# razayunus/ManhattanSLAM

Hardware: AMD Instinct MI355X
Metric: RGB-D frames/sec at 640x480 (ORB+surfel front end) (higher is better)
Workload: dtype u8/i32 (ORB)/f32+f64 (surfel)

## Files before the change

### manhattanslam_amd/csrc/msl_sf_superpixel.hip

```cpp

#include "msl_sf.h"

using namespace msl;
using namespace msl::sf;

namespace {

__device__ __forceinline__ double div100_exact(double x) {
    const double y = 0.01;
    const double q0 = x * y;
    const double q1 = fma(fma(-q0, 100.0, x), y, q0);
    return fma(fma(-q1, 100.0, x), y, q1);
}

constexpr float float_below(float f) { return __builtin_bit_cast(float, __builtin_bit_cast(unsigned, f) - 1u); }
constexpr float HUBER_RANGE_F = (float)HUBER_RANGE, MAX_ANGLE_COS_F = (float)MAX_ANGLE_COS, DEPTH_005_F = 0.05f, DEPTH_01_F = 0.1f;
static_assert((double)HUBER_RANGE_F > HUBER_RANGE && (double)float_below(HUBER_RANGE_F) < HUBER_RANGE, "0.4f is the float next above 0.4");
static_assert((double)MAX_ANGLE_COS_F > MAX_ANGLE_COS && (double)float_below(MAX_ANGLE_COS_F) < MAX_ANGLE_COS, "0.1f is the float next above 0.1");
static_assert((double)DEPTH_005_F > 0.05 && (double)float_below(DEPTH_005_F) < 0.05, "0.05f is the float next above 0.05");
static_assert((double)DEPTH_01_F > 0.1 && (double)float_below(DEPTH_01_F) < 0.1, "0.1f is the float next above 0.1");
__device__ __forceinline__ bool in_huber_band(float r) { return r < HUBER_RANGE_F && r > -HUBER_RANGE_F; }

__device__ __forceinline__ float seq_sum_f32(const float *a, int n, float s) {
    int p = 0;
    for (; p + 8 <= n; p += 8) {
        const float4 u = *reinterpret_cast<const float4 *>(a + p), v = *reinterpret_cast<const float4 *>(a + p + 4);
        s += u.x; s += u.y; s += u.z; s += u.w; s += v.x; s += v.y; s += v.z; s += v.w;
    }
    for (; p < n; p++) s += a[p];
    return s;
}
__device__ __forceinline__ float huber_term_add(float s, float t) {
    return __builtin_isinf(t) ? (float)((double)s + (t > 0 ? HUBER_RANGE : -1 * HUBER_RANGE)) : s + t;
}

__device__ __forceinline__ float row_ror1(float v) {
    return __int_as_float(__builtin_amdgcn_update_dpp(0, __float_as_int(v), 0x121, 0xF, 0xF, false));
}
__device__ __forceinline__ float chain_block_f32(float s, float t) {
#pragma unroll
    for (int q = 0; q < 16; q++) s = row_ror1(s) + t;
    return s;
}
__device__ __forceinline__ float chain_block_huber(float s, float t) {
#pragma unroll
    for (int q = 0; q < 16; q++) s = huber_term_add(row_ror1(s), t);
    return s;
}

__global__ __launch_bounds__(256) void kb_seed_init(SfDev P) {
    const int slot = blockIdx.y;
    const int seedI = blockIdx.x * 256 + threadIdx.x;
    if (seedI >= P.nseeds) return;
    if (seedI == 0) P.wlCount[slot] = 0;
    const FrameDev F = P.frames[slot];
    const int spX = seedI % P.spW, spY = seedI / P.spW;
    int imageX = spX * SP + SP / 2, imageY = spY * SP + SP / 2;
    imageX = imageX < (P.W - 1) ? imageX : (P.W - 1);
    imageY = imageY < (P.H - 1) ? imageY : (P.H - 1);
    msl_seed s;
    memset(&s, 0, sizeof(s));
    P.fused[(size_t)slot * P.flagStride + seedI] = 0;
    if (member_at(P, F, imageY, imageX) != -1) {
        P.seeds[(size_t)slot * P.nseeds + seedI] = s; P.arec[(size_t)slot * P.nseeds + seedI] = assign_rec(s);
        return;
    }
    s.use = 1;
    s.x = (float)imageX; s.y = (float)imageY;
    vec3b(P, F, (float)imageY, (float)imageX, s.r, s.g, s.b);
    s.meanIntensity = gray_at(P, F, imageY, imageX);
    s.meanDepth = depth_at(P, F, imageY, imageX);
    if (s.meanDepth < 0.01) {
        int xb = spX * SP + SP / 2 - SP, yb = spY * SP + SP / 2 - SP;
        int xe = xb + SP * 2, ye = yb + SP * 2;
        xb = xb > 0 ? xb : 0; yb = yb > 0 ? yb : 0;
        xe = xe < P.W - 1 ? xe : P.W - 1; ye = ye < P.H - 1 ? ye : P.H - 1;
        bool found = false;
        for (int j = yb; j < ye && !found; j++)
            for (int i = xb; i < xe; i++) {
                const float d = depth_at(P, F, j, i);
                if (d > 0.01) { s.meanDepth = d; found = true; break; }
            }
    }
    P.seeds[(size_t)slot * P.nseeds + seedI] = s;
    P.arec[(size_t)slot * P.nseeds + seedI] = assign_rec(s);
}

constexpr int ASSIGN_NY = 2;
__global__ __launch_bounds__(256) void kb_assign(SfDev P, int it, int nSlots, int nbx, int nby) {
    const int bpr = (nbx + 3) >> 2;
    const int nbyG = (nby + ASSIGN_NY - 1) / ASSIGN_NY;
    int slot, blk;
    if (!xcd_slot(bpr * nbyG, nSlots, slot, blk)) return;
    if (blk == 0) {
        if (it > 0 && threadIdx.x < 8) P.changed[slot * 8 + threadIdx.x] = threadIdx.x == 0 ? 1 : 0;
        if (threadIdx.x >= 64 && threadIdx.x < 64 + NCHUNK) P.chunkAbort[(slot * 2 + (it & 1)) * 16 + threadIdx.x - 64] = 0x7FFFFFFF;
    }
    const int wv = __builtin_amdgcn_readfirstlane((int)(threadIdx.x >> 6));
    const int byg = blk / bpr, bxi = (blk - byg * bpr) * 4 + wv;
    if (bxi >= nbx) return;
    const int bx = bxi - 1, by0 = byg * ASSIGN_NY - 1;
    const bool okx0 = bx >= 0 && bx < P.spW, okx1 = bx + 1 < P.spW;
    const int bxc = min(bx, P.spW - 1);
    const AssignRec *arec = P.arec + (unsigned)slot * (unsigned)P.nseeds;
    AssignRec cr[ASSIGN_NY + 1][2];
    int rowIdx[ASSIGN_NY + 1];
#pragma unroll
    for (int r = 0; r <= ASSIGN_NY; r++) {
        const int rc = min(max(by0 + r, 0), P.spH - 1);
        rowIdx[r] = rc * P.spW + bx;
        const AssignRec *rp = arec + (rc * P.spW + bxc);
        cr[r][0] = rp[0]; cr[r][1] = rp[1];
    }
    const FrameDev F = P.frames[slot];
    unsigned short *index = P.index + (size_t)slot * P.pxStride, *amap = P.amap + (size_t)slot * P.pxStride;
    float *pxInv = P.pxInv + (size_t)slot * P.pxStride;
    unsigned *tmin = P.tmin + (size_t)slot * P.nseeds;
    const int lane = threadIdx.x & 63, lx = lane & 7, ly = lane >> 3;
    const int colI = 8 * bx + 4 + lx;
    const float colF = (float)colI;
    const bool colIn = colI >= 0 && colI < P.W;
    bool inImg[ASSIGN_NY];
    int mem[ASSIGN_NY], cur[ASSIGN_NY];
    float gI[ASSIGN_NY], dIn[ASSIGN_NY];
    unsigned tCur[ASSIGN_NY];
#pragma unroll
    for (int k = 0; k < ASSIGN_NY; k++) {
        const int rowI = 8 * (by0 + k) + 4 + ly;
        inImg[k] = colIn && rowI >= 0 && rowI < P.H && by0 + k + 1 < nby;
        const int rowC = min(max(rowI, 0), P.H - 1), colC = min(max(colI, 0), P.W - 1), pc = rowC * P.W + colC;
        mem[k] = member_at(P, F, rowC, colC);
        gI[k] = gray_at(P, F, rowC, colC);
        dIn[k] = it == 0 ? depth_at(P, F, rowC, colC) : *byte_off(pxInv, 4u * (unsigned)pc);
        cur[k] = it == 0 ? 0 : (int)*byte_off(index, 2u * (unsigned)pc);
    }
#pragma unroll
    for (int k = 0; k < ASSIGN_NY; k++)
        tCur[k] = it == 0 ? 0u : *byte_off(tmin, 4u * (unsigned)cur[k]);
#pragma unroll
    for (int k = 0; k < ASSIGN_NY; k++) {
        const int by = by0 + k;
        if (__ballot(inImg[k]) == 0) continue;
        const bool oky0 = by >= 0 && by < P.spH, oky1 = by + 1 < P.spH;
        const int rowI = 8 * by + 4 + ly;
        const int p = rowI * P.W + colI;
        const bool isPlane = mem[k] != -1;
        const float myIntensity = gI[k];
        float myInvDepth = dIn[k];
        if (it == 0) {
            myInvDepth = 0.0f;
            if (dIn[k] > 0.01) myInvDepth = (float)(1.0 / (double)dIn[k]);
            if (inImg[k] && !isPlane) *byte_off_w(pxInv, 4u * (unsigned)p) = myInvDepth;
        }
        const bool pxHasDepth = myInvDepth > 0;
        const double myInvD = (double)myInvDepth;
        const float rowF = (float)rowI;
        float minDistDepth = 1e6f, minDistNodepth = 1e6f;
        int minSpIndexDepth = -1, minSpIndexNodepth = -1;
        bool allHasDepth = true;
        auto consider = [&](const AssignRec &C, int spIndex, bool use) {
            float nodepthCost = 0;
            const float dist = (C.x - colF) * (C.x - colF) + (C.y - rowF) * (C.y - rowF);
            nodepthCost += dist / ((SP / 2) * (SP / 2));
            const float intensityDiff = C.meanIntensity - myIntensity;
            nodepthCost = (float)((double)nodepthCost + div100_exact((double)(intensityDiff * intensityDiff)));
            const bool has = C.invDepth >= 0 && pxHasDepth;
            const float inverseDepthDiff = (float)(C.invDepth - myInvD);
            const float withDepth = (float)((double)nodepthCost + (double)(inverseDepthDiff * inverseDepthDiff) * 400.0);
            const float depthCost = has ? withDepth : nodepthCost;
            allHasDepth = allHasDepth && (has || !use);
            const bool bd = use && depthCost < minDistDepth, bn = use && nodepthCost < minDistNodepth;
            minDistDepth = bd ? depthCost : minDistDepth; minSpIndexDepth = bd ? spIndex : minSpIndexDepth;
            minDistNodepth = bn ? nodepthCost : minDistNodepth; minSpIndexNodepth = bn ? spIndex : minSpIndexNodepth;
        };
        const bool anyStable = (cr[k][0].stable | cr[k][1].stable | cr[k + 1][0].stable | cr[k + 1][1].stable) != 0;
        if (okx0 && oky0) consider(cr[k][0], rowIdx[k], true);
        if (okx0 && oky1) consider(cr[k + 1][0], rowIdx[k + 1], ly != 0);
        if (okx1 && oky0) consider(cr[k][1], rowIdx[k] + 1, lx != 0);
        if (okx1 && oky1) consider(cr[k + 1][1], rowIdx[k + 1] + 1, lx != 0 && ly != 0);
        const int pick = allHasDepth ? minSpIndexDepth : minSpIndexNodepth;
        if (!inImg[k]) continue;
        if (it == 0) { *byte_off_w(index, 2u * (unsigned)p) = isPlane ? (unsigned short)0 : (unsigned short)(pick >= 0 ? pick : 0); continue; }
        *byte_off_w(amap, 2u * (unsigned)p) = isPlane ? IDX_PLANE : (pick >= 0 ? (unsigned short)pick : IDX_NONE);
        if (!isPlane && pick >= 0) {
            if (tCur[k] == 0) {
                if (anyStable && tmin[pick] > (unsigned)p + 1u) atomicMin(&tmin[pick], (unsigned)p + 1u);
            } else if (pick != cur[k]) {
                P.wl[(size_t)slot * P.pxStride + atomicAdd(&P.wlCount[slot], 1u)] = (unsigned)p;
            }
        }
    }
}

__device__ __forceinline__ bool relax_pixel(unsigned *tmin, const unsigned short *index, const unsigned short *amap, int p) {
    const unsigned short a = amap[p];
    if (a >= IDX_PLANE) return false;
    const unsigned tc = __hip_atomic_load(&tmin[index[p]], __ATOMIC_RELAXED, __HIP_MEMORY_SCOPE_AGENT);
    if (tc == 0 || tc > (unsigned)p) return false;
    if (__hip_atomic_load(&tmin[a], __ATOMIC_RELAXED, __HIP_MEMORY_SCOPE_AGENT) <= (unsigned)p + 1u) return false;
    return atomicMin(&tmin[a], (unsigned)p + 1u) > (unsigned)p + 1u;
}

constexpr int PROP_BLOCKS = 16;
__global__ __launch_bounds__(256) void kb_prop(SfDev P, int round, int nSlots) {
    int slot, blk;
    if (!xcd_slot(PROP_BLOCKS, nSlots, slot, blk)) return;
    if (!P.changed[slot * 8 + round]) return;
    unsigned *tmin = P.tmin + (size_t)slot * P.nseeds;
    const unsigned short *index = P.index + (size_t)slot * P.pxStride, *amap = P.amap + (size_t)slot * P.pxStride;
    const unsigned *wl = P.wl + (size_t)slot * P.pxStride;
    const unsigned nwl = P.wlCount[slot];
    bool any = false;
    for (unsigned e = blk * 256 + threadIdx.x; e < nwl; e += PROP_BLOCKS * 256) any |= relax_pixel(tmin, index, amap, (int)wl[e]);
    if (any) P.changed[slot * 8 + round + 1] = 1;
}

__global__ __launch_bounds__(1024) void kb_prop_finish(SfDev P) {
    __shared__ int s_ch;
    const int slot = blockIdx.x;
    if (threadIdx.x == 0) s_ch = P.changed[slot * 8 + PROP_ROUNDS];
    __syncthreads();
    unsigned *tmin = P.tmin + (size_t)slot * P.nseeds;
    const unsigned short *index = P.index + (size_t)slot * P.pxStride, *amap = P.amap + (size_t)slot * P.pxStride;
    const unsigned *wl = P.wl + (size_t)slot * P.pxStride;
    const unsigned nwl = P.wlCount[slot];
    while (s_ch) {
        __syncthreads();
        if (threadIdx.x == 0) s_ch = 0;
        __syncthreads();
        bool any = false;
        for (unsigned e = threadIdx.x; e < nwl; e += 1024) any |= relax_pixel(tmin, index, amap, (int)wl[e]);
        if (any) s_ch = 1;
        __syncthreads();
    }
}

constexpr int PROP_LDS_MAX_SEEDS = 36 * 1024;
__global__ __launch_bounds__(256) void kb_prop_lds(SfDev P) {
    extern __shared__ unsigned s_t[];
    const int slot = blockIdx.x;
    const unsigned nwl = P.wlCount[slot];
// ... 160 lines not shown
                const bool own = rowOk && (!STRADDLE || col >= col0) && col >= xb && col < xe && idq[m].v[e] == seedI;
                hd[e] = own && dq[m].v[e] >= DEPTH_01_F;
                if (own) { sumX += col; sumY += j; sumI += gq[m].v[e]; cnt++; }
                c += hd[e] ? 1 : 0;
            }
            const int incl = row_incl_scan(c);
            int o = nd + incl - c;
#pragma unroll
            for (int e = 0; e < 4; e++)
                if (hd[e]) s_depth[g][o++] = dq[m].v[e];
            nd += row_lane_i32<15>(incl);
        }
    }
    USTAMP();
    sumX = row_sum_i32(sumX); sumY = row_sum_i32(sumY); sumI = row_sum_i32(sumI); cnt = row_sum_i32(cnt);
    __builtin_amdgcn_wave_barrier();
    const bool depthLoop = active && cnt != 0 && nd > 0;
    if (l == 0 && active && cnt == 0)
        atomicMin(&P.chunkAbort[(slot * 2 + (it & 1)) * 16 + seed_chunk(seedI, P.nseeds)], seedI);
    const int ndL = depthLoop ? nd : 0;
    const int nblk = rows_max_i32((ndL + 15) >> 4);
    float meanDepth = 0.0f;
    {
        float sd = 0.0f;
        for (int bq = 0; bq < nblk; bq++) {
            const int e = l + 16 * bq;
            sd = chain_block_f32(sd, e < ndL ? s_depth[g][e] : 0.0f);
        }
        const float sumDepth = row_lane_f32<15>(sd);
        if (depthLoop) meanDepth = sumDepth / (float)nd;
    }
    USTAMP();
    bool open = depthLoop;
    for (int newtonI = 0; newtonI < 5; newtonI++) {
        if (!__ballot(open)) break;
        int inr = 0;
        bool tail = false;
        for (int bq = 0; bq < nblk; bq++) {
            const int e = l + 16 * bq;
            if (open && e < ndL) {
                const float residual = meanDepth - s_depth[g][e];
                if (in_huber_band(residual)) inr++; else tail = true;
            }
        }
        inr = row_sum_i32(inr);
        const bool anyTail = __ballot(tail) != 0ull;
        float sa = 0.0f;
        for (int bq = 0; bq < nblk; bq++) {
            const int e = l + 16 * bq;
            float t = 0.0f;
            if (open && e < ndL) {
                const float residual = meanDepth - s_depth[g][e];
                if (in_huber_band(residual)) t = 2 * residual;
                else t = residual > 0 ? __builtin_inff() : -__builtin_inff();
            }
            sa = anyTail ? chain_block_huber(sa, t) : chain_block_f32(sa, t);
        }
        const float sumA = row_lane_f32<15>(sa);
        const float sumB = (float)(2 * inr);
        const float deltaDepth = (float)((double)(-sumA) / ((double)sumB + 10.0));
        if (open) {
            meanDepth = meanDepth + deltaDepth;
            if ((deltaDepth < 0.01 && deltaDepth > -0.01) || newtonI == 4) open = false;
        }
    }
    USTAMP();
    if (active && l == 0) {
        SeedUpd U;
        U.state = cnt == 0 ? 1 : 2; U.cnt = cnt; U.sumI = sumI; U.sumX = sumX; U.sumY = sumY; U.depthLoop = depthLoop ? 1 : 0; U.meanDepth = meanDepth;
        *reinterpret_cast<SeedUpd *>(P.seedsTmp + ((size_t)slot * P.nseeds + seedI)) = U;
    }
#ifdef MSL_FUSE_STAMPS
    USTAMP();
    if (slot == 0 && (threadIdx.x & 63) == 0) {
        for (int q = 1; q < usn; q++) atomicAdd(&P.delList[96 + q], (unsigned)(ust[q] - ust[q - 1]));
        atomicAdd(&P.delList[96], 1u);
    }
#endif
}


__global__ __launch_bounds__(256) void kb_commit_seeds(SfDev P, int it) {
    const int slot = blockIdx.y;
    const int seedI = blockIdx.x * 256 + threadIdx.x;
    if (seedI >= P.nseeds) return;
    if (seedI == 0) P.wlCount[slot] = 0;
    const size_t si = (size_t)slot * P.nseeds + seedI;
    const SeedUpd U = *reinterpret_cast<const SeedUpd *>(P.seedsTmp + si);
    if (U.state == 0) return;
    const int abortAt = P.chunkAbort[(slot * 2 + (it & 1)) * 16 + seed_chunk(seedI, P.nseeds)];
    if (U.state == 1 || seedI > abortAt) {
        P.seeds[si].stable = 0; P.arec[si].stable = 0u; P.tmin[si] = 0u;
        return;
    }
    const FrameDev &F = P.frames[slot];
    static_assert(sizeof(msl_seed) == 64 && offsetof(msl_seed, meanDepth) == 40 && offsetof(msl_seed, r) == 48 && offsetof(msl_seed, stable) == 61, "msl_seed layout");
    uint4 *rec = reinterpret_cast<uint4 *>(P.seeds + si);
    const uint4 w0o = rec[0], w2o = rec[2], w3o = rec[3];
    const float sumIntensityNum = (float)U.cnt;
    const float sumIntensity = (float)U.sumI / sumIntensityNum, mX = (float)U.sumX / sumIntensityNum, mY = (float)U.sumY / sumIntensityNum;
    const float preIntensity = __uint_as_float(w2o.w), preX = __uint_as_float(w0o.x), preY = __uint_as_float(w0o.y);
    int tR = 0, tG = 0, tB = 0;
    vec3b(P, F, mY, mX, tR, tG, tB);
    const float updateDiff = fabsf(preIntensity - sumIntensity) + fabsf(preX - mX) + fabsf(preY - mY);
    const bool tStable = updateDiff < 0.2;
    const float tDepth = U.depthLoop ? U.meanDepth : 0.0f;
    uint4 w0 = w0o, w2 = w2o, w3 = w3o;
    w0.x = __float_as_uint(mX); w0.y = __float_as_uint(mY);
    w2.z = __float_as_uint(tDepth); w2.w = __float_as_uint(sumIntensity);
    w3.x = (unsigned)tR; w3.y = (unsigned)tG; w3.z = (unsigned)tB;
    w3.w = (w3.w & 0x00FF00FFu) | (tStable ? 0x100u : 0u);
    rec[0] = w0; rec[2] = w2; rec[3] = w3;
    P.tmin[si] = tStable ? T_INF : 0u;
    AssignRec a;
    a.x = mX; a.y = mY; a.meanIntensity = sumIntensity; a.stable = tStable ? 1u : 0u;
    a.invDepth = tDepth > 0 ? 1.0 / (double)tDepth : -1.0; a._pad = 0;
    P.arec[si] = a;
}

__device__ __forceinline__ void pixel_normal(const SfDev &P, int row, int col, float myX, float myY, float myZ, float rightDepth,
                                             float downDepth, float cxr, float cx1, float ryr, float ry1,
                                             float &nX, float &nY, float &nZ) {
    nX = nY = nZ = 0.0f;
    if (row < 1 || row > P.H - 2 || col < 1 || col > P.W - 2) return;
    float rightX = cx1 * rightDepth, rightY = ryr * rightDepth, rightZ = rightDepth;
    float downX = cxr * downDepth, downY = ry1 * downDepth, downZ = downDepth;
    if (myZ < DEPTH_01_F || rightZ < DEPTH_01_F || downZ < DEPTH_01_F) return;
    rightX = rightX - myX; rightY = rightY - myY; rightZ = rightZ - myZ;
    downX = downX - myX; downY = downY - myY; downZ = downZ - myZ;
    float normX = rightY * downZ - rightZ * downY;
    float normY = rightZ * downX - rightX * downZ;
    float normZ = rightX * downY - rightY * downX;
    const float normLength = sqrtf(normX * normX + normY * normY + normZ * normZ);
    normX /= normLength; normY /= normLength; normZ /= normLength;
    const float viewAngle = (normX * myX + normY * myY + normZ * myZ) / sqrtf(myX * myX + myY * myY + myZ * myZ);
    if (viewAngle > -MAX_ANGLE_COS_F && viewAngle < MAX_ANGLE_COS_F) return;
    nX = normX; nY = normY; nZ = normZ;
}

template <int CTRL>
__device__ __forceinline__ double dpp_mov_d(double v) {
    const unsigned long long u = __double_as_longlong(v);
    const unsigned lo = (unsigned)__builtin_amdgcn_update_dpp(0, (int)(unsigned)u, CTRL, 0xF, 0xF, true);
    const unsigned hi = (unsigned)__builtin_amdgcn_update_dpp(0, (int)(unsigned)(u >> 32), CTRL, 0xF, 0xF, true);
    return __longlong_as_double(((unsigned long long)hi << 32) | lo);
}
__device__ __forceinline__ double group_sum_d(double v) {
    v += dpp_mov_d<0x128>(v);
    v += dpp_mov_d<0x124>(v);
    v += dpp_mov_d<0x4E>(v);
    v += dpp_mov_d<0xB1>(v);
    return v;
}

struct PlaneFit { int active; float nx, ny, nz, nb, sumX, sumY, sumZ, maxDist; };
static_assert(sizeof(PlaneFit) <= sizeof(msl_surfel), "the hand-over record fits a candidate slot");
constexpr int PLANE_POOL = 24 * 24 + 12 + 2 * 28;
template <bool STRADDLE>
__global__ __launch_bounds__(64) void kb_seed_plane(SfDev P, int nSlots) {
    __shared__ __attribute__((aligned(16))) float s_pool[6][PLANE_POOL];
    __shared__ __attribute__((aligned(16))) double s_h[4][16];
    int slot, blk;
    const int bW = (P.spW + 1) / 2, bH = (P.spH + 1) / 2;
    if (!xcd_slot(bW * bH, nSlots, slot, blk)) return;
#ifdef MSL_FUSE_STAMPS
    unsigned long long sst[14]; int ssn = 0;
#define SECTION_STAMP() sst[ssn++] = __builtin_amdgcn_s_memtime()
#else
#define SECTION_STAMP()
#endif
    SECTION_STAMP();
    const int g = threadIdx.x >> 4, l = threadIdx.x & 15, lane = threadIdx.x;
    const int spX = (blk % bW) * 2 + (g & 1), spY = (blk / bW) * 2 + (g >> 1);
    const bool inRange = spX < P.spW && spY < P.spH;
    const int seedI = inRange ? spY * P.spW + spX : 0;
    const FrameDev F = P.frames[slot];
#ifdef MSL_FUSE_STAMPS
    { unsigned long long a = (unsigned long long)F.depth; asm volatile("" :: "s"(a)); }
    SECTION_STAMP();
#endif
    const unsigned short *index = P.index + (size_t)slot * P.pxStride;
    const msl_seed S = P.seeds[(size_t)slot * P.nseeds + seedI];
#ifdef MSL_FUSE_STAMPS
    asm volatile("" :: "v"(S.x), "v"(S.meanDepth));
    SECTION_STAMP();
#endif
    const int xb = spX * SP + SP / 2 - SP, yb = spY * SP + SP / 2 - SP;
    float maxDist = 0;
    int nvalid = 0, base = 0, poolUsed = 0;
    {
        const int rq = l >> 2, cq = l & 3;
        const int cx0 = xb + 4 * cq;
        const int wrapRow = cx0 < 0 ? -1 : (cx0 >= P.W ? 1 : 0), wcol0 = cx0 - wrapRow * P.W;
        const bool straddle = STRADDLE && cx0 < P.W && cx0 + 3 >= P.W;
        auto elem_wrap = [&](int e) -> int { return (straddle && cx0 + e >= P.W) ? 1 : 0; };
        Quad<unsigned short> idq[4];
        Quad<float> dq[4], ddq[4];
        float dr3[4];
#pragma unroll
        for (int m = 0; m < 4; m++) {
            const int wr = yb + 4 * m + rq + wrapRow;
            const int row = min(max(wr, 0), P.H - 1);
            if (!straddle) {
                idq[m] = load_quad(byte_off(index, 2u * (unsigned)(row * P.W + wcol0)));
                dq[m] = load_quad(byte_off(F.depthG(), (unsigned)row * P.dsB + 4u * (unsigned)wcol0));
                ddq[m] = load_quad(byte_off(F.depthG(), (unsigned)min(row + 1, P.H - 1) * P.dsB + 4u * (unsigned)wcol0));
                dr3[m] = *byte_off(F.depthG(), (unsigned)row * P.dsB + 4u * (unsigned)min(wcol0 + 4, P.W - 1));
            } else {
#pragma unroll
                for (int e = 0; e < 4; e++) {
                    const int we = elem_wrap(e), col = cx0 + e - we * P.W, rowe = min(max(wr + we, 0), P.H - 1);
                    idq[m].v[e] = index[(size_t)rowe * P.W + col];
                    dq[m].v[e] = F.depthG()[(size_t)rowe * P.dstride + col];
                    ddq[m].v[e] = F.depthG()[(size_t)min(rowe + 1, P.H - 1) * P.dstride + col];
                }
                dr3[m] = 0.0f;
            }
        }
        if (inRange && (cq == 1 || cq == 2)) {
            uint2 *tex = P.tex + (size_t)slot * P.pxStride;
#pragma unroll
            for (int m = 1; m <= 2; m++) {
                uint4 *t4 = reinterpret_cast<uint4 *>(tex + (size_t)(yb + 4 * m + rq) * P.W + cx0);
                t4[0] = make_uint4(__float_as_uint(dq[m].v[0]), idq[m].v[0], __float_as_uint(dq[m].v[1]), idq[m].v[1]);
                t4[1] = make_uint4(__float_as_uint(dq[m].v[2]), idq[m].v[2], __float_as_uint(dq[m].v[3]), idq[m].v[3]);
            }
        }
        unsigned vm = 0;
        float xd2[4], yd2[4];
#pragma unroll
        for (int e = 0; e < 4; e++) { const float xDiff = (xb + 4 * cq + e) - S.x; xd2[e] = xDiff * xDiff; }
#pragma unroll
        for (int m = 0; m < 4; m++) { const float yDiff = (yb + 4 * m + rq) - S.y; yd2[m] = yDiff * yDiff; }
#pragma unroll
        for (int m = 0; m < 4; m++)
#pragma unroll
            for (int e = 0; e < 4; e++) {
                const int i = xb + 4 * cq + e, jrow = yb + 4 * m + rq;
                const int pixelIndex = jrow * P.W + i;
                const bool own = inRange & (pixelIndex >= 0) & (pixelIndex < P.npx) & (idq[m].v[e] == seedI);
                const float dist = xd2[e] + yd2[m];
                maxDist = (own & (dist > maxDist)) ? dist : maxDist;
                vm |= ((own & (dq[m].v[e] >= DEPTH_005_F)) ? 1u : 0u) << (4 * m + e);
            }
        nvalid = __popc(vm);
        SECTION_STAMP();
        nvalid = row_sum_i32(nvalid);
        {
            const int pad = (nvalid + 3) & ~3;
            const int n0 = __builtin_amdgcn_readlane(pad, 0), n1 = __builtin_amdgcn_readlane(pad, 16), n2 = __builtin_amdgcn_readlane(pad, 32), n3 = __builtin_amdgcn_readlane(pad, 48);
            const int b1 = n0 + ((16 - n0) & 31), b2 = b1 + n1, b3 = b2 + n2 + ((16 - n2) & 31);
            base = g == 0 ? 0 : g == 1 ? b1 : g == 2 ? b2 : b3;
            poolUsed = b3 + n3;
            const int padEnd = g == 0 ? b1 : g == 1 ? b2 : g == 2 ? b3 : b3 + n3;
            for (int q = base + nvalid + l; q < padEnd; q += 16) { s_pool[2][q] = 0.0f; s_pool[3][q] = 0.0f; s_pool[4][q] = 0.0f; s_pool[5][q] = 0.0f; }
        }
        int run = base;
#pragma unroll
        for (int m = 0; m < 4; m++) {
            const unsigned q = (vm >> (4 * m)) & 0xFu;
            const int c = __popc(q);
            const int incl = row_incl_scan(c);
            int o = run + incl - c;
            const int rc = ((yb + 4 * m + rq + wrapRow) << 16) | wcol0;
#pragma unroll
            for (int e = 0; e < 4; e++)
                if (q & (1u << e)) {
                    float right = e < 3 ? dq[m].v[e < 3 ? e + 1 : 3] : dr3[m];
                    int rce = rc + e;
                    if (straddle) {
                        const int we = elem_wrap(e), col = cx0 + e - we * P.W, rowe = yb + 4 * m + rq + we;
                        rce = (rowe << 16) | col;
                        right = F.depthG()[(size_t)rowe * P.dstride + min(col + 1, P.W - 1)];
                    }
                    s_pool[2][o] = dq[m].v[e]; s_pool[3][o] = right;
                    s_pool[4][o] = ddq[m].v[e]; s_pool[5][o] = __int_as_float(rce);
                    o++;
                }
            run += row_lane_i32<15>(incl);
        }
    }
    SECTION_STAMP();
    float *const pX = s_pool[0] + base, *const pY = s_pool[1] + base, *const pZ = s_pool[2] + base;
    float *const qX = s_pool[3] + base, *const qY = s_pool[4] + base, *const qZ = s_pool[5] + base;
    maxDist = row_max_f32(maxDist);
    __builtin_amdgcn_wave_barrier();
    for (int e = lane; e < poolUsed; e += 64) {
        const int rc = __float_as_int(s_pool[5][e]);
        const int row = rc >> 16, col = rc & 0xFFFF;
        const float myDepth = s_pool[2][e], rightD = s_pool[3][e], downD = s_pool[4][e];
        const float cxr = P.colX[col], cx1 = P.colX[col + 1], ryr = P.rowY[row], ry1 = P.rowY[row + 1];
        const float x = cxr * myDepth, y = ryr * myDepth;
        float nX, nY, nZ;
        pixel_normal(P, row, col, x, y, myDepth, rightD, downD, cxr, cx1, ryr, ry1, nX, nY, nZ);
        s_pool[0][e] = x; s_pool[1][e] = y;
        s_pool[3][e] = nX; s_pool[4][e] = nY; s_pool[5][e] = nZ;
    }
    __builtin_amdgcn_wave_barrier();
    SECTION_STAMP();
    bool active = inRange && nvalid >= 16;
    float meanDepth = S.meanDepth;
    int ninl = 0;
    {
        int c = 0;
        if (active)
            for (int o = l; o < nvalid; o += 16) {
                const float residual = meanDepth - pZ[o];
                c += in_huber_band(residual) ? 1 : 0;
            }
        ninl = row_sum_i32(c);
    }
    const bool needCompact = active && ninl != nvalid;
    if (__ballot(needCompact)) {
        int w0 = 0;
        for (int t = 0; t < 16; t++) {
            const int o = t * 16 + l;
            bool inl = false;
            float a0 = 0, a1 = 0, a2 = 0, b0 = 0, b1 = 0, b2 = 0;
            if (needCompact && o < nvalid) {
                const float residual = meanDepth - pZ[o];
                inl = in_huber_band(residual);
                a0 = pX[o]; a1 = pY[o]; a2 = pZ[o];
                b0 = qX[o]; b1 = qY[o]; b2 = qZ[o];
            }
            const unsigned gm = (unsigned)((__ballot(inl) >> (g * 16)) & 0xFFFFull);
            __builtin_amdgcn_wave_barrier();
            if (inl) {
                const int w = w0 + __popc(gm & ((1u << l) - 1u));
                pX[w] = a0; pY[w] = a1; pZ[w] = a2;
                qX[w] = b0; qY[w] = b1; qZ[w] = b2;
            }
            w0 += __popc(gm);
            __builtin_amdgcn_wave_barrier();
        }
    }
    SECTION_STAMP();
    if (active && (float)ninl / (float)nvalid < 0.8) active = false;
    float normX, normY, normZ, sumX, sumY, sumZ;
    {
        float acc = 0.0f;
        if (active && l < 6) acc = seq_sum_f32(s_pool[l < 3 ? 3 + l : l - 3] + base, ninl, 0.0f);
        normX = row_lane_f32<0>(acc); normY = row_lane_f32<1>(acc); normZ = row_lane_f32<2>(acc);
        sumX = row_lane_f32<3>(acc); sumY = row_lane_f32<4>(acc); sumZ = row_lane_f32<5>(acc);
        const float normLength = sqrtf(normX * normX + normY * normY + normZ * normZ);
        normX = normX / normLength; normY = normY / normLength; normZ = normZ / normLength;
        sumX /= ninl; sumY /= ninl; sumZ /= ninl;
    }
    SECTION_STAMP();
    float nx = normX, ny = normY, nz = normZ, nb = 0.0f;
    unsigned prevMask = 0xFFFFFFFFu;
    double invl = 0;
    const int ca = l >> 2, cb = l & 3;
    const int r0 = ca == 0 ? 1 : 0, r1 = ca <= 1 ? 2 : 1, r2 = ca <= 2 ? 3 : 2;
    const int c0 = cb == 0 ? 1 : 0, c1 = cb <= 1 ? 2 : 1, c2 = cb <= 2 ? 3 : 2;
    const int tRounds = rows_max_i32(active ? (ninl + 15) >> 4 : 0);
    constexpr int RREG = 6;
    float cpx[RREG], cpy[RREG], cpz[RREG];
#pragma unroll
    for (int t = 0; t < RREG; t++) {
        const int o = l + 16 * t, oc = (active && o < ninl) ? o : 0;
        cpx[t] = cpy[t] = cpz[t] = 0.0f;
        if (t < tRounds) { cpx[t] = pX[oc] - sumX; cpy[t] = pY[oc] - sumY; cpz[t] = pZ[oc] - sumZ; }
    }
    for (int gnI = 0; gnI < 5; gnI++) {
        double J0 = 0, J1 = 0, J2 = 0, J3 = 0;
        unsigned mask = 0;
        auto jstep = [&](int t, float px, float py, float pz) {
            const bool has = l + 16 * t < ninl;
            const float residual = px * nx + py * ny + pz * nz + nb;
            const bool inb = has && in_huber_band(residual);
            mask |= (inb ? 1u : 0u) << t;
            const float r2 = inb ? 2 * residual : 0.0f;
            const float qx = inb ? px : 0.0f, qy = inb ? py : 0.0f, qz = inb ? pz : 0.0f;
            J0 += r2 * qx; J1 += r2 * qy; J2 += r2 * qz; J3 += r2;
            if (__builtin_expect(__ballot(has && !inb) != 0ull, 0)) {
                if (has && residual >= HUBER_RANGE_F) {
                    J0 += HUBER_RANGE * px; J1 += HUBER_RANGE * py; J2 += HUBER_RANGE * pz; J3 += HUBER_RANGE;
                } else if (has && residual <= -HUBER_RANGE_F) {
                    J0 += -1 * HUBER_RANGE * px; J1 += -1 * HUBER_RANGE * py; J2 += -1 * HUBER_RANGE * pz; J3 += -1 * HUBER_RANGE;
                }
            }
        };
        if (active) {
#pragma unroll
            for (int t = 0; t < RREG; t++)
                if (t < tRounds) jstep(t, cpx[t], cpy[t], cpz[t]);
#pragma unroll 1
            for (int t = RREG; t < tRounds; t++) {
                const int o = l + 16 * t, oc = o < ninl ? o : 0;
                jstep(t, pX[oc] - sumX, pY[oc] - sumY, pZ[oc] - sumZ);
            }
        }
        J0 = group_sum_d(J0); J1 = group_sum_d(J1); J2 = group_sum_d(J2); J3 = group_sum_d(J3);
        const bool sameSet = mask == prevMask;
        const unsigned diffGroups = (unsigned)((__ballot(!sameSet) >> (g * 16)) & 0xFFFFull);
        prevMask = mask;
        if (__ballot(diffGroups != 0)) {
            double H00 = 0, H01 = 0, H02 = 0, H03 = 0, H11 = 0, H12 = 0, H13 = 0, H22 = 0, H23 = 0, H33 = 0;
            if (active && diffGroups) {
                auto hstep = [&](int t, float rx, float ry, float rz) {
                    const bool inb = (mask >> t) & 1u;
                    const float px = inb ? rx : 0.0f, py = inb ? ry : 0.0f, pz = inb ? rz : 0.0f;
                    H00 += 2 * px * px; H01 += 2 * px * py; H02 += 2 * px * pz; H03 += 2 * px;
                    H11 += 2 * py * py; H12 += 2 * py * pz; H13 += 2 * py;
                    H22 += 2 * pz * pz; H23 += 2 * pz; H33 += inb ? 2.0 : 0.0;
                };
#pragma unroll
                for (int t = 0; t < RREG; t++)
                    if (t < tRounds) hstep(t, cpx[t], cpy[t], cpz[t]);
#pragma unroll 1
                for (int t = RREG; t < tRounds; t++) {
                    const int oc = ((mask >> t) & 1u) ? l + 16 * t : 0;
                    hstep(t, pX[oc] - sumX, pY[oc] - sumY, pZ[oc] - sumZ);
                }
            }
            H00 = group_sum_d(H00); H01 = group_sum_d(H01); H02 = group_sum_d(H02); H03 = group_sum_d(H03);
            H11 = group_sum_d(H11); H12 = group_sum_d(H12); H13 = group_sum_d(H13);
            H22 = group_sum_d(H22); H23 = group_sum_d(H23); H33 = group_sum_d(H33);
            if (l == 0) {
                double *m = s_h[g];
                m[0] = H00 + 5; m[1] = H01; m[2] = H02; m[3] = H03; m[4] = H01; m[5] = H11 + 5; m[6] = H12; m[7] = H13;
                m[8] = H02; m[9] = H12; m[10] = H22 + 5; m[11] = H23; m[12] = H03; m[13] = H13; m[14] = H23; m[15] = H33 + 5;
            }
            __builtin_amdgcn_wave_barrier();
            {
                const double *m = s_h[g];
#define M_(r, c) m[(c) * 4 + (r)]
                const double d3 = M_(r0, c0) * (M_(r1, c1) * M_(r2, c2) - M_(r1, c2) * M_(r2, c1)) -
                                  M_(r0, c1) * (M_(r1, c0) * M_(r2, c2) - M_(r1, c2) * M_(r2, c0)) +
                                  M_(r0, c2) * (M_(r1, c0) * M_(r2, c1) - M_(r1, c1) * M_(r2, c0));
                const double cof = ((ca + cb) & 1) ? -d3 : d3;
                const double f0 = dpp_mov_d<0x150>(cof), f1 = dpp_mov_d<0x151>(cof), f2 = dpp_mov_d<0x152>(cof), f3 = dpp_mov_d<0x153>(cof);
                const double det = ((M_(0, 0) * f0 + M_(0, 1) * f1) + M_(0, 2) * f2) + M_(0, 3) * f3;
#undef M_
                if (diffGroups) invl = cof / det;
            }
            __builtin_amdgcn_wave_barrier();
        }
        const double prod = invl * (ca == 0 ? J0 : ca == 1 ? J1 : ca == 2 ? J2 : J3);
        const double q0 = prod, q1 = dpp_mov_d<0x12C>(prod), q2 = dpp_mov_d<0x128>(prod), q3 = dpp_mov_d<0x124>(prod);
        const double updr = ((q0 + q1) + q2) + q3;
        const double u0 = dpp_mov_d<0x150>(updr), u1 = dpp_mov_d<0x151>(updr), u2 = dpp_mov_d<0x152>(updr), u3 = dpp_mov_d<0x153>(updr);
        nx = (float)((double)nx - u0); ny = (float)((double)ny - u1); nz = (float)((double)nz - u2); nb = (float)((double)nb - u3);
        SECTION_STAMP();
    }
#ifdef MSL_FUSE_STAMPS
    if (slot == 0 && lane == 0) {
        for (int q = 1; q < ssn; q++) atomicAdd(&P.delList[64 + q], (unsigned)(sst[q] - sst[q - 1]));
        atomicAdd(&P.delList[64], 1u);
    }
#endif
    if (!inRange || l != 0) return;
    PlaneFit T;
    T.active = active ? 1 : 0; T.nx = nx; T.ny = ny; T.nz = nz; T.nb = nb; T.sumX = sumX; T.sumY = sumY; T.sumZ = sumZ; T.maxDist = maxDist;
    __builtin_memcpy(reinterpret_cast<char *>(P.cand + ((size_t)slot * P.nseeds + seedI)), &T, sizeof(T));
}

__global__ __launch_bounds__(256) void kb_seed_finish(SfDev P) {
    const int slot = blockIdx.y;
    const int seedI = blockIdx.x * 256 + threadIdx.x;
    if (seedI >= P.nseeds) return;
    const FrameDev &F = P.frames[slot];
    msl_seed S = P.seeds[(size_t)slot * P.nseeds + seedI];
    PlaneFit T;
    __builtin_memcpy(&T, reinterpret_cast<const char *>(P.cand + ((size_t)slot * P.nseeds + seedI)), sizeof(T));
    const bool active = T.active != 0;
    float nx = T.nx, ny = T.ny, nz = T.nz, nb = T.nb;
    const float sumX = T.sumX, sumY = T.sumY, sumZ = T.sumZ, maxDist = T.maxDist;
    float normX, normY, normZ, meanDepth = S.meanDepth;
    if (active) {
        nb = nb - (nx * sumX + ny * sumY + nz * sumZ);
        {
            const float normLength = sqrtf(nx * nx + ny * ny + nz * nz);
            nx /= normLength; ny /= normLength; nz /= normLength; nb /= normLength;
        }
        normX = nx; normY = ny; normZ = nz;
        const float normB = nb;
        float ax, ay, az;
        back_project(P, S.x, S.y, meanDepth, ax, ay, az);
        double avgX = ax, avgY = ay, avgZ = az;
        {
            const float k = (float)(-1 * (avgX * (double)normX + avgY * (double)normY + avgZ * (double)normZ) - (double)normB);
            avgX += (double)(k * normX); avgY += (double)(k * normY); avgZ += (double)(k * normZ);
            meanDepth = (float)avgZ;
        }
        float viewCos = (float)(-1.0 * ((double)normX * avgX + (double)normY * avgY + (double)normZ * avgZ) / sqrt(avgX * avgX + avgY * avgY + avgZ * avgZ));
        if (viewCos < 0) { viewCos = -viewCos; normX = -normX; normY = -normY; normZ = -normZ; }
        S.normX = normX; S.normY = normY; S.normZ = normZ;
        S.posX = (float)avgX; S.posY = (float)avgY; S.posZ = (float)avgZ;
        S.meanDepth = meanDepth; S.viewCos = viewCos; S.size = sqrtf(maxDist);
        P.seeds[(size_t)slot * P.nseeds + seedI] = S;
    }
    const bool valid = !(S.viewCos < MAX_ANGLE_COS) && !(S.normX == 0 && S.normY == 0 && S.normZ == 0);
    const bool ok = valid && !(S.meanDepth == 0);
    P.candOk[(size_t)slot * P.flagStride + seedI] = ok ? 1 : 0;
    if (!ok) P.fused[(size_t)slot * P.flagStride + seedI] = 2;
    float pw[4] = {0, 0, 0, 0};
    float seedWeight = 0, seedSize = 0;
    if (valid) {
        mul4(F.pose, S.posX, S.posY, S.posZ, 1.0f, pw);
        const float cameraF = (float)(((double)fabsf(P.fx) + (double)fabsf(P.fy)) / 2.0);
        seedSize = S.size * fabsf(S.meanDepth / (cameraF * S.viewCos));
        seedWeight = get_weight(S.meanDepth);
    }
    {
        float4 *fr = P.fuseRec + (size_t)slot * P.nseeds * 3;
        fr[fuserec_index(P.nseeds, seedI, 0)] = make_float4(S.normX, S.normY, S.normZ, S.meanDepth);
        fr[fuserec_index(P.nseeds, seedI, 1)] = make_float4(pw[0], pw[1], pw[2], seedWeight);
        fr[fuserec_index(P.nseeds, seedI, 2)] = make_float4(seedSize, S.meanIntensity, __uint_as_float(rgb_pack(S.r, S.g, S.b)), __uint_as_float(valid ? 1u : 0u));
    }
    if (ok) {
        float nw[3];
        mul3(F.pose, S.normX, S.normY, S.normZ, nw);
        msl_surfel e;
        e.px = pw[0]; e.py = pw[1]; e.pz = pw[2];
        e.r = S.r; e.g = S.g; e.b = S.b;
        e.nx = nw[0]; e.ny = nw[1]; e.nz = nw[2];
        e.size = seedSize;
        e.color = S.meanIntensity;
        e.weight = seedWeight;
        e.updateTimes = 1;
        e.lastUpdate = F.ref;
        P.cand[(size_t)slot * P.nseeds + seedI] = e;
    }
}

__global__ __launch_bounds__(256) void kb_depth_u16(const uint8_t *src, size_t srcStride, size_t srcFrameStride, float *dst, size_t dstFrameStride, int W, int H,
                                                    float factor) {
    const int frame = blockIdx.y;
    const int npx = W * H;
    const uint8_t *sf = src + (size_t)frame * srcFrameStride;
    float *df = dst + (size_t)frame * dstFrameStride;
    for (int i = blockIdx.x * 256 + threadIdx.x; i < npx; i += gridDim.x * 256) {
        const int row = i / W, col = i - row * W;
        const unsigned raw = *reinterpret_cast<const uint16_t *>(sf + (size_t)row * srcStride + 2 * (size_t)col);
        df[i] = (float)raw * factor;
    }
}

__global__ __launch_bounds__(256) void kb_tex_strips(SfDev P) {
    const int slot = blockIdx.y;
    const int wStrip = P.W - P.spW * SP, hStrip = P.H - P.spH * SP;
    const int nRight = wStrip * P.spH * SP, nBottom = P.W * hStrip;
    const int i = blockIdx.x * 256 + threadIdx.x;
    if (i >= nRight + nBottom) return;
    int x, y;
    if (i < nRight) { y = i / wStrip; x = P.spW * SP + i % wStrip; }
    else { const int j = i - nRight; y = P.spH * SP + j / P.W; x = j % P.W; }
    const FrameDev F = P.frames[slot];
    const size_t p = (size_t)y * P.W + x;
    P.tex[(size_t)slot * P.pxStride + p] = make_uint2(__float_as_uint(F.depthG()[(size_t)y * P.dstride + x]), P.index[(size_t)slot * P.pxStride + p]);
}

__global__ __launch_bounds__(64) void k_debug_chain(const float *x, const int *n, float *out, int lists, int huber) {
    const int q = blockIdx.x * 4 + (threadIdx.x >> 4), l = threadIdx.x & 15;
    const int nq = q < lists ? n[q] : 0;
    int nblk = (nq + 15) >> 4;
#pragma unroll
    for (int d = 32; d >= 16; d >>= 1) nblk = max(nblk, __shfl_xor(nblk, d, 64));
    nblk = __builtin_amdgcn_readfirstlane(nblk);
    float s = 0.0f;
    for (int bq = 0; bq < nblk; bq++) {
        const int e = l + 16 * bq;
        const float t = e < nq ? x[(size_t)q * 256 + e] : 0.0f;
        s = huber ? chain_block_huber(s, t) : chain_block_f32(s, t);
    }
    if (q < lists && l == 15) out[q] = s;
}

__global__ void k_debug_div100(const float *x, double *out, long long n) {
    const long long i = (long long)blockIdx.x * 256 + threadIdx.x;
    if (i < n) out[i] = div100_exact((double)(x[i] * x[i]));
}

}

namespace msl {
namespace sf {

void sp_launch_depth_u16(hipStream_t st, const void *src, size_t srcStride, size_t srcFrameStride, float *dst, size_t dstFrameStride, int W, int H, int nFrames,
                         float factor) {
    const unsigned bx = (unsigned)std::min(((long long)W * H + 1023) / 1024, 1024ll);
    hipLaunchKernelGGL(kb_depth_u16, dim3(bx, (unsigned)nFrames), dim3(256), 0, st, (const uint8_t *)src, srcStride, srcFrameStride, dst, dstFrameStride, W, H, factor);
}

bool sp_init_attributes(int nseeds) {
    if (nseeds > PROP_LDS_MAX_SEEDS) return false;
    return hipFuncSetAttribute((const void *)kb_prop_lds, hipFuncAttributeMaxDynamicSharedMemorySize, (int)(sizeof(unsigned) * PROP_LDS_MAX_SEEDS)) == hipSuccess;
}

void sp_launch_stage(KernelProfiler &prof, hipStream_t sp, const SfDev &P, int n, bool propLds) {
    const int W = P.W, H = P.H;
// ... 59 lines not shown
```

Baseline: 25640.

## Pack plane-fit Gauss-Newton sums into f32x2 and merge DPP group reductions

```diff
diff --git a/manhattanslam_amd/csrc/msl_sf_superpixel.hip b/manhattanslam_amd/csrc/msl_sf_superpixel.hip
--- a/manhattanslam_amd/csrc/msl_sf_superpixel.hip
+++ b/manhattanslam_amd/csrc/msl_sf_superpixel.hip
@@ -86,7 +86,7 @@
     P.arec[(size_t)slot * P.nseeds + seedI] = assign_rec(s);
 }
 
-constexpr int ASSIGN_NY = 2;
+constexpr int ASSIGN_NY = 3;
 __global__ __launch_bounds__(256) void kb_assign(SfDev P, int it, int nSlots, int nbx, int nby) {
     const int bpr = (nbx + 3) >> 2;
     const int nbyG = (nby + ASSIGN_NY - 1) / ASSIGN_NY;
@@ -553,10 +553,27 @@
     v += dpp_mov_d<0xB1>(v);
     return v;
 }
+__device__ __forceinline__ double bank_pick_d(int l, unsigned banks, double x, double y) { return ((banks >> (l >> 2)) & 1u) ? x : y; }
+__device__ __forceinline__ double group_sum4_d(int l, double a, double b, double c, double d) {
+    const double ab = bank_pick_d(l, 0x9u, a, b) + dpp_mov_d<0x128>(bank_pick_d(l, 0x9u, b, a));
+    const double cd = bank_pick_d(l, 0x3u, c, d) + dpp_mov_d<0x128>(bank_pick_d(l, 0x3u, d, c));
+    double v = bank_pick_d(l, 0x5u, ab, cd) + dpp_mov_d<0x124>(bank_pick_d(l, 0x5u, cd, ab));
+    v += dpp_mov_d<0x4E>(v);
+    v += dpp_mov_d<0xB1>(v);
+    return v;
+}
+__device__ __forceinline__ double group_sum2_d(int l, double a, double b) {
+    double v = bank_pick_d(l, 0x9u, a, b) + dpp_mov_d<0x128>(bank_pick_d(l, 0x9u, b, a));
+    v += dpp_mov_d<0x124>(v);
+    v += dpp_mov_d<0x4E>(v);
+    v += dpp_mov_d<0xB1>(v);
+    return v;
+}
 
 struct PlaneFit { int active; float nx, ny, nz, nb, sumX, sumY, sumZ, maxDist; };
 static_assert(sizeof(PlaneFit) <= sizeof(msl_surfel), "the hand-over record fits a candidate slot");
 constexpr int PLANE_POOL = 24 * 24 + 12 + 2 * 28;
+typedef float f32x2 __attribute__((ext_vector_type(2)));
 template <bool STRADDLE>
 __global__ __launch_bounds__(64) void kb_seed_plane(SfDev P, int nSlots) {
     __shared__ __attribute__((aligned(16))) float s_pool[6][PLANE_POOL];
@@ -756,12 +773,12 @@
     const int c0 = cb == 0 ? 1 : 0, c1 = cb <= 1 ? 2 : 1, c2 = cb <= 2 ? 3 : 2;
     const int tRounds = rows_max_i32(active ? (ninl + 15) >> 4 : 0);
     constexpr int RREG = 6;
-    float cpx[RREG], cpy[RREG], cpz[RREG];
+    f32x2 cpx[RREG / 2], cpy[RREG / 2], cpz[RREG / 2];
 #pragma unroll
     for (int t = 0; t < RREG; t++) {
         const int o = l + 16 * t, oc = (active && o < ninl) ? o : 0;
-        cpx[t] = cpy[t] = cpz[t] = 0.0f;
-        if (t < tRounds) { cpx[t] = pX[oc] - sumX; cpy[t] = pY[oc] - sumY; cpz[t] = pZ[oc] - sumZ; }
+        cpx[t >> 1][t & 1] = cpy[t >> 1][t & 1] = cpz[t >> 1][t & 1] = 0.0f;
+        if (t < tRounds) { cpx[t >> 1][t & 1] = pX[oc] - sumX; cpy[t >> 1][t & 1] = pY[oc] - sumY; cpz[t >> 1][t & 1] = pZ[oc] - sumZ; }
     }
     for (int gnI = 0; gnI < 5; gnI++) {
         double J0 = 0, J1 = 0, J2 = 0, J3 = 0;
@@ -782,17 +799,36 @@
                 }
             }
         };
+        auto jpair = [&](int t) {
+            const f32x2 px = cpx[t >> 1], py = cpy[t >> 1], pz = cpz[t >> 1];
+            const f32x2 residual = px * nx + py * ny + pz * nz + nb;
+            const bool has0 = l + 16 * t < ninl, has1 = l + 16 * (t + 1) < ninl;
+            const bool inb0 = has0 && in_huber_band(residual.x), inb1 = has1 && in_huber_band(residual.y);
+            if (__builtin_expect(__ballot((has0 && !inb0) || (has1 && !inb1)) != 0ull, 0)) {
+                jstep(t, px.x, py.x, pz.x); jstep(t + 1, px.y, py.y, pz.y);
+                return;
+            }
+            mask |= ((inb0 ? 1u : 0u) | (inb1 ? 2u : 0u)) << t;
+            const f32x2 tw = 2 * residual;
+            const f32x2 r2 = {inb0 ? tw.x : 0.0f, inb1 ? tw.y : 0.0f};
+            const f32x2 qx = {inb0 ? px.x : 0.0f, inb1 ? px.y : 0.0f}, qy = {inb0 ? py.x : 0.0f, inb1 ? py.y : 0.0f}, qz = {inb0 ? pz.x : 0.0f, inb1 ? pz.y : 0.0f};
+            const f32x2 jx = r2 * qx, jy = r2 * qy, jz = r2 * qz;
+            J0 += jx.x; J1 += jy.x; J2 += jz.x; J3 += r2.x;
+            J0 += jx.y; J1 += jy.y; J2 += jz.y; J3 += r2.y;
+        };
         if (active) {
 #pragma unroll
-            for (int t = 0; t < RREG; t++)
-                if (t < tRounds) jstep(t, cpx[t], cpy[t], cpz[t]);
+            for (int t = 0; t < RREG; t += 2) {
+                if (t + 1 < tRounds) jpair(t);
+                else if (t < tRounds) jstep(t, cpx[t >> 1].x, cpy[t >> 1].x, cpz[t >> 1].x);
+            }
 #pragma unroll 1
             for (int t = RREG; t < tRounds; t++) {
                 const int o = l + 16 * t, oc = o < ninl ? o : 0;
                 jstep(t, pX[oc] - sumX, pY[oc] - sumY, pZ[oc] - sumZ);
             }
         }
-        J0 = group_sum_d(J0); J1 = group_sum_d(J1); J2 = group_sum_d(J2); J3 = group_sum_d(J3);
+        const double Jca = group_sum4_d(l, J0, J2, J1, J3);
         const bool sameSet = mask == prevMask;
         const unsigned diffGroups = (unsigned)((__ballot(!sameSet) >> (g * 16)) & 0xFFFFull);
         prevMask = mask;
@@ -806,22 +842,38 @@
                     H11 += 2 * py * py; H12 += 2 * py * pz; H13 += 2 * py;
                     H22 += 2 * pz * pz; H23 += 2 * pz; H33 += inb ? 2.0 : 0.0;
                 };
-#pragma unroll
-                for (int t = 0; t < RREG; t++)
-                    if (t < tRounds) hstep(t, cpx[t], cpy[t], cpz[t]);
+                auto hpair = [&](int t) {
+                    const bool inb0 = (mask >> t) & 1u, inb1 = (mask >> (t + 1)) & 1u;
+                    const f32x2 rx = cpx[t >> 1], ry = cpy[t >> 1], rz = cpz[t >> 1];
+                    const f32x2 px = {inb0 ? rx.x : 0.0f, inb1 ? rx.y : 0.0f}, py = {inb0 ? ry.x : 0.0f, inb1 ? ry.y : 0.0f}, pz = {inb0 ? rz.x : 0.0f, inb1 ? rz.y : 0.0f};
+                    const f32x2 px2 = 2 * px, py2 = 2 * py, pz2 = 2 * pz;
+                    const f32x2 hxx = px2 * px, hxy = px2 * py, hxz = px2 * pz, hyy = py2 * py, hyz = py2 * pz, hzz = pz2 * pz;
+                    H00 += hxx.x; H01 += hxy.x; H02 += hxz.x; H03 += px2.x;
+                    H11 += hyy.x; H12 += hyz.x; H13 += py2.x;
+                    H22 += hzz.x; H23 += pz2.x; H33 += inb0 ? 2.0 : 0.0;
+                    H00 += hxx.y; H01 += hxy.y; H02 += hxz.y; H03 += px2.y;
+                    H11 += hyy.y; H12 += hyz.y; H13 += py2.y;
+                    H22 += hzz.y; H23 += pz2.y; H33 += inb1 ? 2.0 : 0.0;
+                };
+#pragma unroll
+                for (int t = 0; t < RREG; t += 2) {
+                    if (t + 1 < tRounds) hpair(t);
+                    else if (t < tRounds) hstep(t, cpx[t >> 1].x, cpy[t >> 1].x, cpz[t >> 1].x);
+                }
 #pragma unroll 1
                 for (int t = RREG; t < tRounds; t++) {
                     const int oc = ((mask >> t) & 1u) ? l + 16 * t : 0;
                     hstep(t, pX[oc] - sumX, pY[oc] - sumY, pZ[oc] - sumZ);
                 }
             }
-            H00 = group_sum_d(H00); H01 = group_sum_d(H01); H02 = group_sum_d(H02); H03 = group_sum_d(H03);
-            H11 = group_sum_d(H11); H12 = group_sum_d(H12); H13 = group_sum_d(H13);
-            H22 = group_sum_d(H22); H23 = group_sum_d(H23); H33 = group_sum_d(H33);
-            if (l == 0) {
+            const double hA = group_sum4_d(l, H00, H02, H01, H03), hB = group_sum4_d(l, H11, H13, H12, H22), hC = group_sum2_d(l, H23, H33);
+            if ((l & 3) == 0) {
                 double *m = s_h[g];
-                m[0] = H00 + 5; m[1] = H01; m[2] = H02; m[3] = H03; m[4] = H01; m[5] = H11 + 5; m[6] = H12; m[7] = H13;
-                m[8] = H02; m[9] = H12; m[10] = H22 + 5; m[11] = H23; m[12] = H03; m[13] = H13; m[14] = H23; m[15] = H33 + 5;
+                const int b = l >> 2;
+                auto put = [&](int r, int c, double h) { const double e = r == c ? h + 5 : h; m[c * 4 + r] = e; m[r * 4 + c] = e; };
+                put(0, b, hA);
+                put(b == 3 ? 2 : 1, b == 3 ? 2 : 1 + b, hB);
+                if ((b & 1) == 0) put(2 + (b >> 1), 3, hC);
             }
             __builtin_amdgcn_wave_barrier();
             {
@@ -838,7 +890,7 @@
             }
             __builtin_amdgcn_wave_barrier();
         }
-        const double prod = invl * (ca == 0 ? J0 : ca == 1 ? J1 : ca == 2 ? J2 : J3);
+        const double prod = invl * Jca;
         const double q0 = prod, q1 = dpp_mov_d<0x12C>(prod), q2 = dpp_mov_d<0x128>(prod), q3 = dpp_mov_d<0x124>(prod);
         const double updr = ((q0 + q1) + q2) + q3;
         const double u0 = dpp_mov_d<0x150>(updr), u1 = dpp_mov_d<0x151>(updr), u2 = dpp_mov_d<0x152>(updr), u3 = dpp_mov_d<0x153>(updr);
```

Result: no change. 25810, median of 6 (+0.7%).
